# tschnz/Live-Video-Magnification

Hardware: NVIDIA H100
Metric: 1080p frames/sec (Laplace, 6-level) (higher is better)
Workload: dtype f32

## Files before the change

### live-video-magnification_b200/csrc/mc_core.cu

```cuda
#include <algorithm>
#include <cmath>
#include <cstdio>
#include <cstring>
#include <deque>
#include <new>
#include <string>
#include <vector>

#include "../../include/magcore_b200.h"
#include "mc_internal.h"
#include "mc_modes.h"

using namespace mc;

namespace {
thread_local std::string g_create_error;

struct Slot {
    uint8_t *h_in = nullptr, *h_out = nullptr;
    uint8_t *d_in = nullptr, *d_out = nullptr;
    size_t bytes = 0;
    cudaEvent_t ev_in = nullptr, ev_k = nullptr, ev_done = nullptr;
    int produced = 0;
    std::vector<uint8_t> lane_produced;
    uint8_t* user_out = nullptr;
    size_t user_out_step = 0;
    bool direct_out = false;
    int w = 0, h = 0, c = 0;
    bool nv12 = false;
    mc_nv12 user_nv12{};
};
}

struct mc_handle {
    int device = 0;
    int lanes = 1;
    cudaStream_t stream = nullptr, s_in = nullptr, s_out = nullptr;
    DeviceTables tables;
    std::string err;
    uint64_t launches = 0;

    int t_mode = MC_MODE_NONE, t_levels = -1, t_channels = -1, t_w = 0, t_h = 0;
    int t_down = 1, t_roi = 0;
    float t_rx = 0.f, t_ry = 0.f, t_rw = 1.f, t_rh = 1.f;

    bool faithful0 = false, keep_float = false, profile = false, use_tma = true, prefetch_state = true, band_from_state = true, analysis_only = false;
    int ingest_warps = 1;
    int egress_strip = 20;
    int lane_groups = 0;
    Profiler prof;
    int depth = 3;

    MotionMode motion;
    ColorMode color;
    RieszMode riesz;

    float* float_out = nullptr;
    size_t float_out_floats = 0;

    uint8_t *c_raw = nullptr, *c_pre = nullptr, *c_gray = nullptr, *c_out = nullptr;
    size_t c_raw_b = 0, c_pre_b = 0, c_gray_b = 0, c_out_b = 0;
    void* c_tabs = nullptr;
    size_t c_tabs_b = 0;

    uint8_t *k_in = nullptr, *k_out = nullptr;
    size_t k_in_b = 0, k_out_b = 0;

    uint8_t *n_in = nullptr, *n_out = nullptr, *n_flags = nullptr;
    size_t n_in_b = 0, n_out_b = 0, n_flags_b = 0;

    std::vector<Slot> slots;
    std::deque<int> inflight;
    int next_slot = 0;

    std::vector<uint8_t> has_state, hold, ops;
    std::vector<uint8_t> lane_produced;
    uint8_t* d_ops = nullptr;
};

namespace {
thread_local int g_inject_throw = 0;

inline void debug_maybe_throw() {
    if (g_inject_throw > 0 && --g_inject_throw == 0) throw std::bad_alloc();
}

void reset_modes(mc_handle* h);
void tracker_reset(mc_handle* h);

mc_status on_exception(mc_handle* h) noexcept {
    const char* what = "unknown C++ exception";
    std::string buf;
    try { throw; }
    catch (const std::bad_alloc&) { what = "out of host memory (std::bad_alloc)"; }
    catch (const std::exception& e) {
        try { buf = std::string("C++ exception: ") + e.what(); what = buf.c_str(); } catch (...) {}
    }
    catch (...) {}
    try {
        if (h) {
            h->err = what;
// ... 342 lines not shown
    if (h->n_in) cudaFree(h->n_in);
    if (h->n_out) cudaFree(h->n_out);
    if (h->n_flags) cudaFree(h->n_flags);
    if (h->tables.lab_lut) cudaFree(h->tables.lab_lut);
    if (h->tables.inv_gamma) cudaFree(h->tables.inv_gamma);
    if (h->d_ops) cudaFree(h->d_ops);
    if (h->stream) cudaStreamDestroy(h->stream);
    if (h->s_in) cudaStreamDestroy(h->s_in);
    if (h->s_out) cudaStreamDestroy(h->s_out);
    delete h;
} catch (...) {}

void mc_debug_inject_exception(int nth) { g_inject_throw = nth; }

mc_status mc_reset(mc_handle* h) try {
    if (!h) return MC_ERR_INVALID;
    CK(cudaSetDevice(h->device));
    CK(cudaStreamSynchronize(h->stream));
    reset_modes(h);
    tracker_reset(h);
    return MC_OK;
} catch (...) { return on_exception(h); }

mc_status mc_restart_lane(mc_handle* h, int lane) try {
    if (!h) return MC_ERR_INVALID;
    if (lane < 0 || lane >= h->lanes) { h->err = "lane out of range"; return MC_ERR_INVALID; }
    if (h->lanes == 1) return mc_reset(h);
    h->has_state[(size_t)lane] = 0;
    return MC_OK;
} catch (...) { return on_exception(h); }

mc_status mc_hold_lane(mc_handle* h, int lane, int hold) try {
    if (!h) return MC_ERR_INVALID;
    if (lane < 0 || lane >= h->lanes) { h->err = "lane out of range"; return MC_ERR_INVALID; }
    h->hold[(size_t)lane] = hold != 0;
    return MC_OK;
} catch (...) { return on_exception(h); }

mc_status mc_lane_produced(mc_handle* h, uint8_t* produced, int n) try {
    if (!h || !produced) return MC_ERR_INVALID;
    if (n != h->lanes) { h->err = "n must equal the handle's lanes"; return MC_ERR_INVALID; }
    std::memcpy(produced, h->lane_produced.data(), (size_t)n);
    return MC_OK;
} catch (...) { return on_exception(h); }

mc_status mc_set_option(mc_handle* h, const char* key, int value) try {
    if (!h || !key) return MC_ERR_INVALID;
    if (!std::strcmp(key, "faithful_level0")) { h->faithful0 = value != 0; return MC_OK; }
    if (!std::strcmp(key, "keep_float_output")) { h->keep_float = value != 0; return MC_OK; }
    if (!std::strcmp(key, "profile_kernels")) { h->profile = value != 0; return MC_OK; }
    if (!std::strcmp(key, "use_tma")) { h->use_tma = value != 0; return MC_OK; }
    if (!std::strcmp(key, "prefetch_state")) { h->prefetch_state = value != 0; return MC_OK; }
    if (!std::strcmp(key, "lane_groups")) { h->lane_groups = value < 0 ? 0 : value; return MC_OK; }
    if (!std::strcmp(key, "egress_strip")) { h->egress_strip = value == 1 ? 20 : value; return MC_OK; }
    if (!std::strcmp(key, "ingest_warps")) { h->ingest_warps = value; return MC_OK; }
    if (!std::strcmp(key, "band_from_state")) { h->band_from_state = value != 0; return MC_OK; }
    if (!std::strcmp(key, "analysis_only")) { h->analysis_only = value != 0; return MC_OK; }
    if (!std::strcmp(key, "pipeline_depth")) {
        if (value < 1 || value > 16 || !h->inflight.empty()) { h->err = "bad pipeline_depth"; return MC_ERR_INVALID; }
        h->depth = value;
        free_slots(h);
        return MC_OK;
    }
    h->err = std::string("unknown option ") + key;
    return MC_ERR_INVALID;
} catch (...) { return on_exception(h); }

void* mc_stream(mc_handle* h) { return h ? (void*)h->stream : nullptr; }
uint64_t mc_launch_count(mc_handle* h) { return h ? h->launches : 0; }
int mc_pipeline_depth(mc_handle* h) { return h ? h->depth : 0; }

const char* mc_last_error(mc_handle* h) { return h ? h->err.c_str() : g_create_error.c_str(); }

mc_status mc_sync(mc_handle* h) try {
    if (!h) return MC_ERR_INVALID;
    CK(cudaSetDevice(h->device));
    CK(cudaStreamSynchronize(h->stream));
    return MC_OK;
} catch (...) { return on_exception(h); }

mc_status mc_process_device(mc_handle* h, const uint8_t* d_in, int width, int height, int channels, size_t in_step,
                            const mc_params* p, uint8_t* d_out, size_t out_step, int* produced) try {
    if (!h || !produced) return MC_ERR_INVALID;
    CK(cudaSetDevice(h->device));
    return process_device_impl(h, d_in, width, height, channels, in_step, p, d_out, out_step, produced, h->lane_produced.data());
} catch (...) { return on_exception(h); }

mc_status mc_submit(mc_handle* h, const uint8_t* in, int width, int height, int channels, size_t in_step,
                    const mc_params* p, uint8_t* out, size_t out_step) try {
    if (!h || !p) return MC_ERR_INVALID;
    CK(cudaSetDevice(h->device));
    if ((int)h->inflight.size() >= h->depth) { h->err = "pipeline full: call mc_collect first"; return MC_ERR_INVALID; }
    const bool have = in != nullptr && width > 0 && height > 0 && (channels == 1 || channels == 3);
    const size_t row = have ? (size_t)width * channels : 0;
    const size_t bytes = row * (size_t)(have ? height : 0) * h->lanes;
    if (have && in_step < row) { h->err = "step too small"; return MC_ERR_INVALID; }
    mc_status st = ensure_slots(h, std::max<size_t>(bytes, 1));
    if (st != MC_OK) return st;
    const int si = h->next_slot;
    Slot& s = h->slots[(size_t)si];
    s.w = width; s.h = height; s.c = channels; s.produced = 0;
    s.user_out = out; s.user_out_step = out_step; s.direct_out = false; s.nv12 = false;
    if (have && out && out_step < row) { h->err = "out_step too small"; return MC_ERR_INVALID; }
    if (!have) {
        int produced = 0;
        st = process_device_impl(h, nullptr, 0, 0, channels, 0, p, nullptr, 0, &produced, s.lane_produced.data());
        if (st != MC_OK) return st;
// ... 504 lines not shown
```

### live-video-magnification_b200/csrc/mc_laplace.cu

```cuda
#include <cuda.h>

#include "mc_internal.h"
#include "mc_tma.cuh"

namespace mc {

namespace {

__device__ __forceinline__ void prefetch_l1(const void* p) {
#if !defined(MC_CUDA_EMU)
    asm volatile("prefetch.global.L1 [%0];" ::"l"(p));
#else
    (void)p;
#endif
}

constexpr float kInv256 = 1.0f / 256.0f;
constexpr float kInv64 = 1.0f / 64.0f;

__device__ __forceinline__ float down5(float a, float b, float c, float d, float e) {
    return c * 6.0f + (b + d) * 4.0f + a + e;
}

__device__ __forceinline__ float up3(float a, float b, float c) { return __fadd_rn(__fmaf_rn(b, 6.0f, a), c); }
// ... 671 lines not shown
        }
        *reinterpret_cast<float4*>(out + o) = v;
    }
}

constexpr int E2W = 20, E2H = 12;
constexpr int E2P = 20;

struct EgressArgs {
    const uint8_t* in; size_t in_step, in_lane_stride;
    const int16_t* lab; int pitch16; size_t plane16;
    uint8_t* out; size_t out_step, out_lane_stride;
    int w0, h0;
    const float4* gtab; LabInvCoeffs coeffs;
    BandSrc m1; Level l1;
    BandSrc c2; Level l2;
    float chroma;
    float* fout;
    const uint8_t* ops;
    int first_only;
};

__device__ __forceinline__ bool egress_skips(const EgressArgs& a, int lane) {
    const int op = lane_op(a.ops, lane);
    return op == LANE_HOLD || (a.first_only && op == LANE_RUN);
}

template <int C> struct EgressIn;
template <> struct EgressIn<3> { short4 L, A, B; };
template <> struct EgressIn<1> { uint32_t g; };

template <int C>
__device__ __forceinline__ EgressIn<C> egress_load(const EgressArgs& a, int lane, int gy, int gx);
template <>
__device__ __forceinline__ EgressIn<3> egress_load<3>(const EgressArgs& a, int lane, int gy, int gx) {
    const int16_t* lp = a.lab + (size_t)(lane * 3) * a.plane16 + (size_t)gy * a.pitch16 + gx;
    EgressIn<3> r;
    r.L = __ldg(reinterpret_cast<const short4*>(lp));
    r.A = __ldg(reinterpret_cast<const short4*>(lp + a.plane16));
    r.B = __ldg(reinterpret_cast<const short4*>(lp + 2 * a.plane16));
    return r;
}
template <>
__device__ __forceinline__ EgressIn<1> egress_load<1>(const EgressArgs& a, int lane, int gy, int gx) {
    const uint8_t* p = a.in + (size_t)lane * a.in_lane_stride + (size_t)gy * a.in_step + gx;
    EgressIn<1> r;
    r.g = 0;
#pragma unroll
    for (int i = 0; i < 4; ++i)
        if (gx + i < a.w0) r.g |= (uint32_t)__ldg(p + i) << (8 * i);
    return r;
}

template <int C>
__device__ __forceinline__ void egress_convert(const EgressArgs& a, uint8_t* q, float* f, int gx, const EgressIn<C>& in, const float (&up)[C][4]);
template <>
__device__ __forceinline__ void egress_convert<3>(const EgressArgs& a, uint8_t* q, float* f, int gx, const EgressIn<3>& in, const float (&up)[3][4]) {
    uint8_t o8[12];
    float of[12];
    const float chroma64 = a.chroma * kInv64;
    const short vL[4] = {in.L.x, in.L.y, in.L.z, in.L.w}, vA[4] = {in.A.x, in.A.y, in.A.z, in.A.w}, vB[4] = {in.B.x, in.B.y, in.B.z, in.B.w};
#pragma unroll
    for (int i = 0; i < 4; ++i) {
        float L = (float)vL[i] * (100.0f / 16384.0f);
        float A = fmaf((float)vA[i], 1.0f / 64.0f, -128.0f);
        float B = fmaf((float)vB[i], 1.0f / 64.0f, -128.0f);
        if (a.m1.a) {
            L = __fmaf_rn(up[0][i], kInv64, L);
            A = __fadd_rn(A, __fmul_rn(up[1][i], chroma64));
            B = __fadd_rn(B, __fmul_rn(up[2][i], chroma64));
        }
        float ob, og, orr;
        lab_to_bgr_fast(L, A, B, a.coeffs, a.gtab, ob, og, orr);
        of[3 * i] = ob; of[3 * i + 1] = og; of[3 * i + 2] = orr;
        o8[3 * i] = unit01_to_u8(ob); o8[3 * i + 1] = unit01_to_u8(og); o8[3 * i + 2] = unit01_to_u8(orr);
    }
    if (gx + 4 <= a.w0 && ((reinterpret_cast<uintptr_t>(q) & 3) == 0)) {
#pragma unroll
        for (int wd = 0; wd < 3; ++wd)
            reinterpret_cast<uint32_t*>(q)[wd] = (uint32_t)o8[4 * wd] | ((uint32_t)o8[4 * wd + 1] << 8) |
                                                 ((uint32_t)o8[4 * wd + 2] << 16) | ((uint32_t)o8[4 * wd + 3] << 24);
    } else {
#pragma unroll
        for (int i = 0; i < 12; ++i)
            if (gx + i / 3 < a.w0) q[i] = o8[i];
    }
    if (f) {
#pragma unroll
        for (int i = 0; i < 12; ++i)
            if (gx + i / 3 < a.w0) f[i] = of[i];
    }
}
template <>
__device__ __forceinline__ void egress_convert<1>(const EgressArgs& a, uint8_t* q, float* f, int gx, const EgressIn<1>& in, const float (&up)[1][4]) {
    uint8_t o8[4];
    float of[4];
#pragma unroll
    for (int i = 0; i < 4; ++i) {
        float v = u8_to_unit((uint8_t)((in.g >> (8 * i)) & 0xff));
        if (a.m1.a) v = __fmaf_rn(up[0][i], kInv64, v);
        of[i] = v;
        o8[i] = unit_to_u8(v);
    }
    if (gx + 4 <= a.w0 && ((reinterpret_cast<uintptr_t>(q) & 3) == 0)) {
        *reinterpret_cast<uint32_t*>(q) = (uint32_t)o8[0] | ((uint32_t)o8[1] << 8) | ((uint32_t)o8[2] << 16) | ((uint32_t)o8[3] << 24);
    } else {
#pragma unroll
        for (int i = 0; i < 4; ++i)
            if (gx + i < a.w0) q[i] = o8[i];
    }
    if (f) {
#pragma unroll
        for (int i = 0; i < 4; ++i)
            if (gx + i < a.w0) f[i] = of[i];
    }
}

template <int C>
__device__ __forceinline__ void egress_pixels(const EgressArgs& a, int lane, int gy, int gx, const float (&up)[C][4]) {
    const EgressIn<C> in = egress_load<C>(a, lane, gy, gx);
    uint8_t* q = a.out + (size_t)lane * a.out_lane_stride + (size_t)gy * a.out_step + (size_t)gx * C;
    float* f = a.fout ? a.fout + (((size_t)lane * a.h0 + gy) * a.w0 + gx) * C : nullptr;
    egress_convert<C>(a, q, f, gx, in, up);
}

template <int C>
// ... 53 lines not shown
                if (from_state) v[ch] = band_of(v[ch], __ldg(pl[ch] + o1), g1);
            }
            if (has2) {
                const int ky = (y1 >> 1) - by2;
                const bool odd = y1 & 1;
#pragma unroll
                for (int ch = 0; ch < C; ++ch) {
                    const float r0 = sT[ch][ky - 1][j], r1 = sT[ch][ky][j], r2 = sT[ch][ky + 1][j];
                    v[ch] = __fmaf_rn(odd ? up2(r1, r2) : up3(r0, r1, r2), kInv64, v[ch]);
                }
            }
#pragma unroll
            for (int ch = 0; ch < C; ++ch) sD[ch][k][j] = v[ch];
        }
        __syncthreads();
    }
    const int tx = threadIdx.x & 15, ty = threadIdx.x >> 4;
    const int gx = x0 + 4 * tx;
    if (gx >= a.w0) return;
    float up[C][2][4];
    if (a.m1.a) {
#pragma unroll
        for (int ch = 0; ch < C; ++ch) {
            float e[3][4];
#pragma unroll
            for (int q = 0; q < 3; ++q) {
                const float2 p0 = *reinterpret_cast<const float2*>(&sD[ch][ty + q][2 * tx]);
                const float2 p1 = *reinterpret_cast<const float2*>(&sD[ch][ty + q][2 * tx + 2]);
                e[q][0] = up3(p0.x, p0.y, p1.x);
                e[q][1] = up2(p0.y, p1.x);
                e[q][2] = up3(p0.y, p1.x, p1.y);
                e[q][3] = up2(p1.x, p1.y);
            }
#pragma unroll
            for (int i = 0; i < 4; ++i) {
                up[ch][0][i] = up3(e[0][i], e[1][i], e[2][i]);
                up[ch][1][i] = up2(e[1][i], e[2][i]);
            }
        }
    }
#pragma unroll
    for (int ry = 0; ry < 2; ++ry) {
        const int gy = y0 + 2 * ty + ry;
        if (gy >= a.h0) continue;
        float upr[C][4];
#pragma unroll
        for (int ch = 0; ch < C; ++ch)
#pragma unroll
            for (int i = 0; i < 4; ++i) upr[ch][i] = up[ch][ry][i];
        egress_pixels<C>(a, lane, gy, gx, upr);
    }
}

template <int C>
__device__ __forceinline__ EgressIn<C> egress_rows3(const int16_t* const (&p)[C], size_t off);
template <>
__device__ __forceinline__ EgressIn<3> egress_rows3<3>(const int16_t* const (&p)[3], size_t off) {
    EgressIn<3> r;
    r.L = __ldg(reinterpret_cast<const short4*>(p[0] + off));
    r.A = __ldg(reinterpret_cast<const short4*>(p[1] + off));
    r.B = __ldg(reinterpret_cast<const short4*>(p[2] + off));
    return r;
}
template <>
__device__ __forceinline__ EgressIn<1> egress_rows3<1>(const int16_t* const (&)[1], size_t) { return EgressIn<1>{0}; }
template <int C>
__device__ __forceinline__ EgressIn<C> egress_row1(const uint8_t* row, int gx, int w0);
template <>
__device__ __forceinline__ EgressIn<1> egress_row1<1>(const uint8_t* row, int gx, int w0) {
    EgressIn<1> r;
    r.g = 0;
#pragma unroll
    for (int i = 0; i < 4; ++i)
        if (gx >= 0 && gx + i < w0) r.g |= (uint32_t)__ldg(row + gx + i) << (8 * i);
    return r;
}
template <>
__device__ __forceinline__ EgressIn<3> egress_row1<3>(const uint8_t*, int, int) { return EgressIn<3>{}; }

constexpr int EG_ROWS = 64;

template <int C> struct StripM1 { float2 h[C], l[C]; };
template <int C> struct StripH2 { float v[C], vb[C], vr[C], vrb[C]; };

template <int C, int MINB>
__global__ void __launch_bounds__(32, MINB) k_egress_strip(const EgressArgs a) {
    const unsigned full = 0xffffffffu;
    const int lane_id = threadIdx.x;
    const int lane = blockIdx.z;
    const int gx = blockIdx.x * DS_COLS - 4 + lane_id * 4;
    const int f0 = blockIdx.y * EG_ROWS;
    if (f0 >= a.h0 || egress_skips(a, lane)) return;
    const int f_end = min(f0 + EG_ROWS, a.h0);
    const bool px_owner = lane_id >= 1 && lane_id <= 30 && gx < a.w0;
    if (!a.m1.a) {
        float zero[C][4];
#pragma unroll
        for (int ch = 0; ch < C; ++ch)
#pragma unroll
            for (int i = 0; i < 4; ++i) zero[ch][i] = 0.0f;
        if (px_owner)
            for (int gy = f0; gy < f_end; ++gy) egress_pixels<C>(a, lane, gy, gx, zero);
        return;
    }
    const int w1 = a.l1.w, h1 = a.l1.h, w2 = a.l2.w, h2 = a.l2.h;
    const int x1a = gx >> 1, x2 = gx >> 2;
    const bool has2 = a.c2.a != nullptr, from_state = a.m1.b != nullptr, st2 = a.c2.b != nullptr;
    const float g1 = a.m1.gain, g2 = a.c2.gain;
    const int x1l = x1a < 0 ? 0 : (x1a >= w1 ? ((w1 - 1) & ~1) : x1a);
    const int x2l = x2 < 0 ? 0 : (x2 >= w2 ? w2 - 1 : x2);
    const int x2r = x2l + 1 >= w2 ? w2 - 1 : x2l + 1;
    const int gxl = px_owner ? gx : 0;
    size_t base1[C], base2[C];
#pragma unroll
    for (int ch = 0; ch < C; ++ch) {
        base1[ch] = (size_t)(lane * C + ch) * a.l1.plane + x1l;
        base2[ch] = (size_t)(lane * C + ch) * a.l2.plane;
    }

    auto row1 = [&](int y1) { return (size_t)(y1 < h1 ? y1 : h1 - 1) * a.l1.pitch; };
    auto ld_m1 = [&](int y1) {
        StripM1<C> m;
        const size_t ro = row1(y1);
#pragma unroll
        for (int ch = 0; ch < C; ++ch) {
            m.h[ch] = __ldg(reinterpret_cast<const float2*>(a.m1.a + base1[ch] + ro));
            m.l[ch] = from_state ? __ldg(reinterpret_cast<const float2*>(a.m1.b + base1[ch] + ro)) : make_float2(0.f, 0.f);
        }
        return m;
    };
    auto pf_m1 = [&](int y1) {
        const size_t ro = row1(y1);
#pragma unroll
        for (int ch = 0; ch < C; ++ch) {
            prefetch_l1(a.m1.a + base1[ch] + ro);
            if (from_state) prefetch_l1(a.m1.b + base1[ch] + ro);
        }
    };
    auto ld_h2 = [&](int y2) {
        StripH2<C> r;
        const size_t ro = (size_t)upsrc(y2, h2) * a.l2.pitch;
#pragma unroll
        for (int ch = 0; ch < C; ++ch) {
            r.v[ch] = r.vb[ch] = r.vr[ch] = r.vrb[ch] = 0.f;
            if (has2) {
                r.v[ch] = __ldg(a.c2.a + base2[ch] + ro + x2l);
                if (st2) r.vb[ch] = __ldg(a.c2.b + base2[ch] + ro + x2l);
                if (lane_id == 31) {
                    r.vr[ch] = __ldg(a.c2.a + base2[ch] + ro + x2r);
                    if (st2) r.vrb[ch] = __ldg(a.c2.b + base2[ch] + ro + x2r);
                }
            }
        }
        return r;
    };
    auto pf_h2 = [&](int y2) {
        const size_t ro = (size_t)upsrc(y2, h2) * a.l2.pitch;
        if (has2) {
#pragma unroll
            for (int ch = 0; ch < C; ++ch) {
                prefetch_l1(a.c2.a + base2[ch] + ro + x2l);
                if (st2) prefetch_l1(a.c2.b + base2[ch] + ro + x2l);
            }
        }
    };
    auto pf_in = [&](int gy) {
        if (C == 3) {
            const int16_t* lp = a.lab + (size_t)(lane * 3) * a.plane16 + (size_t)gy * a.pitch16 + gxl;
            prefetch_l1(lp); prefetch_l1(lp + a.plane16); prefetch_l1(lp + 2 * a.plane16);
        } else {
            prefetch_l1(a.in + (size_t)lane * a.in_lane_stride + (size_t)gy * a.in_step + gxl);
        }
    };
    __shared__ float2 sH[3][C][32];
    __shared__ float4 sE[3][C][32];
    auto slot = [](int r) { return (r + 3) % 3; };
    auto expand_h2 = [&](const StripH2<C>& in, int i) {
        const int sl = slot(i);
#pragma unroll
        for (int ch = 0; ch < C; ++ch) {
            const float v = st2 ? band_of(in.v[ch], in.vb[ch], g2) : in.v[ch];
            float l = __shfl_up_sync(full, v, 1), r = __shfl_down_sync(full, v, 1);
            if (lane_id == 31) r = st2 ? band_of(in.vr[ch], in.vrb[ch], g2) : in.vr[ch];
            if (x2 == 0) l = r;
            if (x2 + 1 >= w2) r = v;
            sH[sl][ch][lane_id] = make_float2(up3(l, v, r), up2(v, r));
        }
    };
    auto cur1_row = [&](const StripM1<C>& m, int y1, float (&E)[C][4]) {
        const bool odd = y1 & 1;
        const int i = y1 >> 1;
        const int sp = slot(odd ? i : i - 1), sq = slot(odd ? i + 1 : i), sr = slot(i + 1);
#pragma unroll
        for (int ch = 0; ch < C; ++ch) {
            float ca = m.h[ch].x, cb = m.h[ch].y;
            if (from_state) {
                ca = band_of(ca, m.l[ch].x, g1);
                cb = band_of(cb, m.l[ch].y, g1);
            }
            if (has2) {
                const float2 p = sH[sp][ch][lane_id], q = sH[sq][ch][lane_id], r = sH[sr][ch][lane_id];
                ca = __fmaf_rn(odd ? up2(p.x, q.x) : up3(p.x, q.x, r.x), kInv64, ca);
                cb = __fmaf_rn(odd ? up2(p.y, q.y) : up3(p.y, q.y, r.y), kInv64, cb);
            }
            if (x1a + 1 >= w1) cb = ca;
            float left = __shfl_up_sync(full, cb, 1), right = __shfl_down_sync(full, ca, 1);
            if (x1a == 0) left = cb;
            if (x1a + 2 >= w1) right = cb;
            E[ch][0] = up3(left, ca, cb);
            E[ch][1] = up2(ca, cb);
            E[ch][2] = up3(ca, cb, right);
            E[ch][3] = up2(cb, right);
        }
    };
    auto put_E = [&](int j, const float (&E)[C][4]) {
        const int sl = slot(j);
#pragma unroll
        for (int ch = 0; ch < C; ++ch) sE[sl][ch][lane_id] = make_float4(E[ch][0], E[ch][1], E[ch][2], E[ch][3]);
    };

    const int j0 = f0 >> 1;
    {
        const int ic = j0 >> 1;
        const StripH2<C> ra = ld_h2(ic - 1), rb = ld_h2(ic), rc = ld_h2(ic + 1);
        const StripM1<C> mp = ld_m1(j0 > 0 ? j0 - 1 : 1), m0 = ld_m1(j0);
        pf_m1(j0 + 1);
        pf_in(2 * j0);
        pf_in(min(2 * j0 + 1, a.h0 - 1));
        expand_h2(ra, ic - 1);
        expand_h2(rb, ic);
        expand_h2(rc, ic + 1);
        float E[C][4];
        if (j0 > 0) { cur1_row(mp, j0 - 1, E); put_E(j0 - 1, E); }
        cur1_row(m0, j0, E);
        put_E(j0, E);
    }
    const int j_end = (f_end + 1) >> 1;
    const size_t st1 = (size_t)a.l1.pitch, st16 = (size_t)a.pitch16;
    const float* ph[C];
    const float* pl[C];
    const int16_t* pin[C];
#pragma unroll
    for (int ch = 0; ch < C; ++ch) {
        const size_t ro = row1(j0 + 1);
        ph[ch] = a.m1.a + base1[ch] + ro;
        pl[ch] = from_state ? a.m1.b + base1[ch] + ro : ph[ch];
        pin[ch] = C == 3 ? a.lab + (size_t)(lane * 3 + ch) * a.plane16 + (size_t)(2 * j0) * st16 + gxl : nullptr;
    }
    const uint8_t* pg = C == 1 ? a.in + (size_t)lane * a.in_lane_stride + (size_t)(2 * j0) * a.in_step : nullptr;
    uint8_t* pq = a.out + (size_t)lane * a.out_lane_stride + (size_t)(2 * j0) * a.out_step + (size_t)gx * C;
    int sm = slot(j0 - 1), s0 = slot(j0), sp = slot(j0 + 1);
    for (int j = j0; j < j_end; ++j) {
        const int jn = j + 1;
        const bool two = 2 * j + 1 < f_end;
        StripM1<C> cm;
#pragma unroll
        for (int ch = 0; ch < C; ++ch) {
            cm.h[ch] = __ldg(reinterpret_cast<const float2*>(ph[ch]));
            cm.l[ch] = from_state ? __ldg(reinterpret_cast<const float2*>(pl[ch])) : make_float2(0.f, 0.f);
        }
        StripH2<C> chh;
        if (!(jn & 1) && jn < h1) chh = ld_h2((jn >> 1) + 1);
        EgressIn<C> in0, in1;
        if (C == 3) {
            in0 = egress_rows3<C>(pin, 0);
            in1 = egress_rows3<C>(pin, two ? st16 : 0);
        } else {
            in0 = egress_row1<C>(pg, gx, a.w0);
            in1 = egress_row1<C>(two ? pg + a.in_step : pg, gx, a.w0);
        }
        if (jn < j_end) {
            const bool adv1 = jn + 1 < h1;
            if (jn & 1) pf_h2(((jn + 1) >> 1) + 1);
#pragma unroll
            for (int ch = 0; ch < C; ++ch) {
                if (adv1) { ph[ch] += st1; pl[ch] += st1; }
                prefetch_l1(ph[ch]);
                if (from_state) prefetch_l1(pl[ch]);
                if (C == 3) {
                    pin[ch] += 2 * st16;
                    prefetch_l1(pin[ch]);
                    if (2 * jn + 1 < a.h0) prefetch_l1(pin[ch] + st16);
                }
            }
            if (C == 1) { pg += 2 * a.in_step; prefetch_l1(pg + gxl); }
        }
        float Ep[C][4];
        if (jn >= h1) {
#pragma unroll
            for (int ch = 0; ch < C; ++ch) {
                const float4 e = sE[s0][ch][lane_id];
                Ep[ch][0] = e.x; Ep[ch][1] = e.y; Ep[ch][2] = e.z; Ep[ch][3] = e.w;
            }
        } else {
            if (!(jn & 1)) expand_h2(chh, (jn >> 1) + 1);
            cur1_row(cm, jn, Ep);
        }
#pragma unroll
        for (int ch = 0; ch < C; ++ch) sE[sp][ch][lane_id] = make_float4(Ep[ch][0], Ep[ch][1], Ep[ch][2], Ep[ch][3]);
        if (j == 0) {
#pragma unroll
            for (int ch = 0; ch < C; ++ch) sE[sm][ch][lane_id] = make_float4(Ep[ch][0], Ep[ch][1], Ep[ch][2], Ep[ch][3]);
        }
        if (px_owner) {
            float up[C][4], t0[C][4];
#pragma unroll
            for (int ch = 0; ch < C; ++ch) {
                const float4 em = sE[sm][ch][lane_id], e0 = sE[s0][ch][lane_id];
                t0[ch][0] = e0.x; t0[ch][1] = e0.y; t0[ch][2] = e0.z; t0[ch][3] = e0.w;
                up[ch][0] = up3(em.x, e0.x, Ep[ch][0]);
                up[ch][1] = up3(em.y, e0.y, Ep[ch][1]);
                up[ch][2] = up3(em.z, e0.z, Ep[ch][2]);
                up[ch][3] = up3(em.w, e0.w, Ep[ch][3]);
            }
            float* f = a.fout ? a.fout + (((size_t)lane * a.h0 + 2 * j) * a.w0 + gx) * C : nullptr;
            egress_convert<C>(a, pq, f, gx, in0, up);
            if (two) {
#pragma unroll
                for (int ch = 0; ch < C; ++ch)
#pragma unroll
                    for (int i = 0; i < 4; ++i) up[ch][i] = up2(t0[ch][i], Ep[ch][i]);
                egress_convert<C>(a, pq + a.out_step, f ? f + (size_t)a.w0 * C : nullptr, gx, in1, up);
            }
        }
        pq += 2 * a.out_step;
        const int t = sm; sm = s0; s0 = sp; sp = t;
    }
}

__global__ void k_copy(float* __restrict__ dst, const float* __restrict__ src, size_t n) {
    for (size_t i = (size_t)blockIdx.x * blockDim.x + threadIdx.x; i < n; i += (size_t)gridDim.x * blockDim.x)
        dst[i] = src[i];
}

inline unsigned cdiv(int a, int b) { return (unsigned)((a + b - 1) / b); }

}

typedef CUresult (*TensorMapEncodeFn)(CUtensorMap*, CUtensorMapDataType, cuuint32_t, void*, const cuuint64_t*, const cuuint64_t*,
                                      const cuuint32_t*, const cuuint32_t*, CUtensorMapInterleave, CUtensorMapSwizzle,
                                      CUtensorMapL2promotion, CUtensorMapFloatOOBfill);
static TensorMapEncodeFn tensor_map_encoder() {
    static const TensorMapEncodeFn fn = [] {
        void* p = nullptr;
        cudaDriverEntryPointQueryResult qres;
        if (cudaGetDriverEntryPoint("cuTensorMapEncodeTiled", &p, cudaEnableDefault, &qres) != cudaSuccess || !p) {
            cudaGetLastError();
            p = nullptr;
        }
        return reinterpret_cast<TensorMapEncodeFn>(p);
    }();
    return fn;
}

bool make_tensor_map_box(void* out_map, const float* base, const Level& l, int planes, int box_w, int box_h) {
    const TensorMapEncodeFn encode = tensor_map_encoder();
    if (!encode) return false;
    const cuuint64_t dims[3] = {(cuuint64_t)l.w, (cuuint64_t)l.h, (cuuint64_t)planes};
    const cuuint64_t strides[2] = {(cuuint64_t)l.pitch * sizeof(float), (cuuint64_t)l.plane * sizeof(float)};
    const cuuint32_t box[3] = {(cuuint32_t)box_w, (cuuint32_t)box_h, 1u};
    const cuuint32_t estr[3] = {1u, 1u, 1u};
    const CUresult r = encode(reinterpret_cast<CUtensorMap*>(out_map), CU_TENSOR_MAP_DATA_TYPE_FLOAT32, 3, const_cast<float*>(base),
                              dims, strides, box, estr, CU_TENSOR_MAP_INTERLEAVE_NONE, CU_TENSOR_MAP_SWIZZLE_NONE,
                              CU_TENSOR_MAP_L2_PROMOTION_L2_128B, CU_TENSOR_MAP_FLOAT_OOB_FILL_NONE);
    return r == CUDA_SUCCESS;
}

bool make_level_tensor_map(void* out_map, const float* base, const Level& l, int planes, bool state_tile) {
    return make_tensor_map_box(out_map, base, l, planes, state_tile ? TW : GW, state_tile ? TH : GH);
}

cudaError_t launch_lab16(const FrameIO& io, const DeviceTables& tb, int16_t* lab, int pitch16, size_t plane16,
                         cudaStream_t s, float* l_f32, int l_pitch, size_t l_plane) {
    const int aligned = (reinterpret_cast<uintptr_t>(io.in) % 4 == 0) && (io.in_step % 4 == 0) && (io.in_lane_stride % 4 == 0);
    dim3 grid(cdiv(cdiv(io.w, 4), 256), io.h, io.lanes);
    k_lab16<<<grid, 256, 0, s>>>(io.in, io.in_step, io.in_lane_stride, io.w, io.h, tb.lab_lut, lab, pitch16, plane16, aligned, l_f32, l_pitch, l_plane, io.ops);
    return cudaGetLastError();
}
// ... 25 lines not shown
    k.ops = a.ops;
    k.in_vec_ok = a.in_kind == IN_U8 ? ((reinterpret_cast<uintptr_t>(a.g) % 4 == 0) && (a.in_row % 4 == 0) && (a.in_plane % 4 == 0)) : 1;
    return k;
}

cudaError_t launch_level_clip(const LevelArgs& a, int frames, cudaStream_t s) {
    const LevelKArgs k = level_kargs(a);
    dim3 grid(cdiv(a.lf.w, TW), cdiv(a.lf.h, TH), a.planes);
    static const CUtensorMap dummy{};
    const CUtensorMap* tg = reinterpret_cast<const CUtensorMap*>(a.tmap);
    if (a.in_kind == IN_F32 && tg) k_level_clip<IN_F32, true><<<grid, 256, 0, s>>>(k, frames, a.planes, *tg);
    else if (a.in_kind == IN_F32) k_level_clip<IN_F32, false><<<grid, 256, 0, s>>>(k, frames, a.planes, dummy);
    else if (a.in_kind == IN_LAB16) k_level_clip<IN_LAB16, false><<<grid, 256, 0, s>>>(k, frames, a.planes, dummy);
    else k_level_clip<IN_U8, false><<<grid, 256, 0, s>>>(k, frames, a.planes, dummy);
    return cudaGetLastError();
}

cudaError_t launch_level(const LevelArgs& a, cudaStream_t s) {
    const LevelKArgs k = level_kargs(a);
    dim3 grid(cdiv(a.lf.w, TW), cdiv(a.lf.h, TH), a.planes);
    static const CUtensorMap dummy{};
    const CUtensorMap* tg = reinterpret_cast<const CUtensorMap*>(a.tmap);
    if (a.in_kind == IN_F32 && tg && a.tmap_hi && a.tmap_lo)
        k_level<IN_F32, true, true><<<grid, 256, 0, s>>>(k, *tg, *reinterpret_cast<const CUtensorMap*>(a.tmap_hi),
                                                          *reinterpret_cast<const CUtensorMap*>(a.tmap_lo));
    else if (a.in_kind == IN_F32 && tg) k_level<IN_F32, true, false><<<grid, 256, 0, s>>>(k, *tg, dummy, dummy);
    else if (a.in_kind == IN_F32) k_level<IN_F32, false, false><<<grid, 256, 0, s>>>(k, dummy, dummy, dummy);
    else if (a.in_kind == IN_LAB16) k_level<IN_LAB16, false, false><<<grid, 256, 0, s>>>(k, dummy, dummy, dummy);
    else k_level<IN_U8, false, false><<<grid, 256, 0, s>>>(k, dummy, dummy, dummy);
    return cudaGetLastError();
}

cudaError_t launch_down(const LevelArgs& a, cudaStream_t s) {
    DownArgs k;
    k.g = a.g; k.in_plane = a.in_plane; k.in_row = a.in_row; k.channels = a.channels;
    for (int i = 0; i < 3; ++i) { k.sc[i] = a.sc[i]; k.of[i] = a.of[i]; }
    k.lf = a.lf; k.lc = a.lc; k.g_next = a.g_next;
    k.ops = a.ops;
    k.in_vec_ok = a.in_kind == IN_U8 ? ((reinterpret_cast<uintptr_t>(a.g) % 4 == 0) && (a.in_row % 4 == 0) && (a.in_plane % 4 == 0)) : 1;
    dim3 grid(cdiv(a.lf.w, DS_COLS), cdiv(a.lc.h, DS_ROWS * DS_WARPS), a.planes);
    if (a.in_kind == IN_F32) k_down_strip<IN_F32><<<grid, 32 * DS_WARPS, 0, s>>>(k);
    else if (a.in_kind == IN_LAB16) k_down_strip<IN_LAB16><<<grid, 32 * DS_WARPS, 0, s>>>(k);
    else k_down_strip<IN_U8><<<grid, 32 * DS_WARPS, 0, s>>>(k);
    return cudaGetLastError();
}

cudaError_t launch_collapse(const Level& lf, const Level& lc, const BandSrc& fine, const BandSrc& coarse, float* out, int planes,
                            cudaStream_t s, const uint8_t* ops, int channels) {
    dim3 grid(cdiv(lf.w, TW), cdiv(lf.h, TH), planes);
    k_collapse<<<grid, 256, 0, s>>>(lf, lc, fine, coarse, out, ops, channels);
    return cudaGetLastError();
}

cudaError_t launch_egress(const FrameIO& io, const DeviceTables& tb, const int16_t* lab, int pitch16, size_t plane16,
                          const BandSrc& m1, const Level& l1, const BandSrc& c2, const Level& l2, float chroma,
                          float* fout, cudaStream_t s, int strip, bool first_only) {
    EgressArgs a;
    a.in = io.in; a.in_step = io.in_step; a.in_lane_stride = io.in_lane_stride;
    a.lab = lab; a.pitch16 = pitch16; a.plane16 = plane16;
    a.out = io.out; a.out_step = io.out_step; a.out_lane_stride = io.out_lane_stride;
    a.w0 = io.w; a.h0 = io.h;
    a.gtab = tb.inv_gamma; a.coeffs = tb.inv_coeffs;
    a.m1 = m1; a.l1 = l1; a.c2 = c2; a.l2 = l2; a.chroma = chroma; a.fout = fout;
    a.ops = io.ops; a.first_only = first_only ? 1 : 0;
    if (strip) {
        dim3 grid(cdiv(io.w, DS_COLS), cdiv(io.h, EG_ROWS), io.lanes);
        if (io.channels != 3) k_egress_strip<1, 24><<<grid, 32, 0, s>>>(a);
        else if (strip == 16) k_egress_strip<3, 16><<<grid, 32, 0, s>>>(a);
        else if (strip == 24) k_egress_strip<3, 24><<<grid, 32, 0, s>>>(a);
        else k_egress_strip<3, 20><<<grid, 32, 0, s>>>(a);
    } else {
        dim3 grid(cdiv(io.w, TW), cdiv(io.h, TH), io.lanes);
        if (io.channels == 3) k_egress<3><<<grid, 256, 0, s>>>(a);
        else k_egress<1><<<grid, 256, 0, s>>>(a);
    }
    return cudaGetLastError();
}

cudaError_t launch_copy_planes(float* dst, const float* src, size_t n, cudaStream_t s) {
    unsigned blocks = (unsigned)((n + 255) / 256);
    if (blocks > 132 * 8) blocks = 132 * 8;
    if (blocks == 0) blocks = 1;
    k_copy<<<blocks, 256, 0, s>>>(dst, src, n);
    return cudaGetLastError();
}

}
```

Measured before the change: 17040.

## Restructure egress strip kernel with warp-uniform dark-gamma fallback and int offsets

Reworks the strip egress kernel. Gamma is now computed with a fast exp2/log2 path, and the spline table lookup runs only when some lane in the warp has a dark value, checked with a warp vote. Pointer arithmetic moves to 32-bit offsets, the float output path becomes a compile-time template flag, and all lanes compute the upsampled values uniformly to avoid divergence. The default strip launch bound also changes from 20 to 16; the risk is extra register pressure and a possible change in numeric behaviour near the dark threshold.

```diff
diff --git a/live-video-magnification_b200/csrc/mc_core.cu b/live-video-magnification_b200/csrc/mc_core.cu
--- a/live-video-magnification_b200/csrc/mc_core.cu
+++ b/live-video-magnification_b200/csrc/mc_core.cu
@@ -46,7 +46,7 @@
 
     bool faithful0 = false, keep_float = false, profile = false, use_tma = true, prefetch_state = true, band_from_state = true, analysis_only = false;
     int ingest_warps = 1;
-    int egress_strip = 20;
+    int egress_strip = 16;
     int lane_groups = 0;
     Profiler prof;
     int depth = 3;
@@ -495,7 +495,7 @@
     if (!std::strcmp(key, "use_tma")) { h->use_tma = value != 0; return MC_OK; }
     if (!std::strcmp(key, "prefetch_state")) { h->prefetch_state = value != 0; return MC_OK; }
     if (!std::strcmp(key, "lane_groups")) { h->lane_groups = value < 0 ? 0 : value; return MC_OK; }
-    if (!std::strcmp(key, "egress_strip")) { h->egress_strip = value == 1 ? 20 : value; return MC_OK; }
+    if (!std::strcmp(key, "egress_strip")) { h->egress_strip = value == 1 ? 16 : value; return MC_OK; }
     if (!std::strcmp(key, "ingest_warps")) { h->ingest_warps = value; return MC_OK; }
     if (!std::strcmp(key, "band_from_state")) { h->band_from_state = value != 0; return MC_OK; }
     if (!std::strcmp(key, "analysis_only")) { h->analysis_only = value != 0; return MC_OK; }
diff --git a/live-video-magnification_b200/csrc/mc_laplace.cu b/live-video-magnification_b200/csrc/mc_laplace.cu
--- a/live-video-magnification_b200/csrc/mc_laplace.cu
+++ b/live-video-magnification_b200/csrc/mc_laplace.cu
@@ -747,6 +747,53 @@
     return r;
 }
 
+__device__ __forceinline__ void egress_lab_in(short l, short av, short bv, bool motion, float u0, float u1, float u2,
+                                              float chroma64, float& L, float& A, float& B) {
+    L = (float)l * (100.0f / 16384.0f);
+    A = fmaf((float)av, 1.0f / 64.0f, -128.0f);
+    B = fmaf((float)bv, 1.0f / 64.0f, -128.0f);
+    if (motion) {
+        L = __fmaf_rn(u0, kInv64, L);
+        A = __fadd_rn(A, __fmul_rn(u1, chroma64));
+        B = __fadd_rn(B, __fmul_rn(u2, chroma64));
+    }
+}
+
+constexpr float kGammaDark = 8.0f / 1024.0f;
+
+__device__ __forceinline__ void lab_lin(float L, float a, float b, const LabInvCoeffs& k, float& vb, float& vg, float& vr) {
+    const float y_lin = L * (1.0f / 903.3f);
+    const float fy_lin = 7.787f * y_lin + 16.0f / 116.0f;
+    const float fy_cub = (L + 16.0f) * (1.0f / 116.0f);
+    const bool lo = L <= 8.0f;
+    const float fy = lo ? fy_lin : fy_cub;
+    const float Y = lo ? y_lin : fy_cub * fy_cub * fy_cub;
+    const float fx = a * (1.0f / 500.0f) + fy;
+    const float fz = fy - b * (1.0f / 200.0f);
+    const float fth = 6.0f / 29.0f;
+    const float X = fx <= fth ? (fx - 16.0f / 116.0f) * (1.0f / 7.787f) : fx * fx * fx;
+    const float Z = fz <= fth ? (fz - 16.0f / 116.0f) * (1.0f / 7.787f) : fz * fz * fz;
+    vb = __saturatef(__fmaf_rn(k.c[2], Z, __fmaf_rn(k.c[1], Y, __fmul_rn(k.c[0], X))));
+    vg = __saturatef(__fmaf_rn(k.c[5], Z, __fmaf_rn(k.c[3], X, __fmul_rn(k.c[4], Y))));
+    vr = __saturatef(__fmaf_rn(k.c[8], Z, __fmaf_rn(k.c[6], X, __fmul_rn(k.c[7], Y))));
+}
+
+__device__ __forceinline__ float gamma_fast(float v) { return fmaf(1.055f, mc_ex2(mc_lg2(v) * (1.0f / 2.4f)), -0.055f); }
+
+__device__ __forceinline__ void lab_to_bgr_egress(float L, float a, float b, const LabInvCoeffs& k, const float4* __restrict__ gtab,
+                                                  float& ob, float& og, float& orr) {
+    float vb, vg, vr;
+    lab_lin(L, a, b, k, vb, vg, vr);
+    ob = gamma_fast(vb);
+    og = gamma_fast(vg);
+    orr = gamma_fast(vr);
+    if (fminf(vb, fminf(vg, vr)) < kGammaDark) {
+        if (vb < kGammaDark) ob = spline_gamma(vb, gtab);
+        if (vg < kGammaDark) og = spline_gamma(vg, gtab);
+        if (vr < kGammaDark) orr = spline_gamma(vr, gtab);
+    }
+}
+
 template <int C>
 __device__ __forceinline__ void egress_convert(const EgressArgs& a, uint8_t* q, float* f, int gx, const EgressIn<C>& in, const float (&up)[C][4]);
 template <>
@@ -757,16 +804,10 @@
     const short vL[4] = {in.L.x, in.L.y, in.L.z, in.L.w}, vA[4] = {in.A.x, in.A.y, in.A.z, in.A.w}, vB[4] = {in.B.x, in.B.y, in.B.z, in.B.w};
 #pragma unroll
     for (int i = 0; i < 4; ++i) {
-        float L = (float)vL[i] * (100.0f / 16384.0f);
-        float A = fmaf((float)vA[i], 1.0f / 64.0f, -128.0f);
-        float B = fmaf((float)vB[i], 1.0f / 64.0f, -128.0f);
-        if (a.m1.a) {
-            L = __fmaf_rn(up[0][i], kInv64, L);
-            A = __fadd_rn(A, __fmul_rn(up[1][i], chroma64));
-            B = __fadd_rn(B, __fmul_rn(up[2][i], chroma64));
-        }
+        float L, A, B;
+        egress_lab_in(vL[i], vA[i], vB[i], a.m1.a != nullptr, up[0][i], up[1][i], up[2][i], chroma64, L, A, B);
         float ob, og, orr;
-        lab_to_bgr_fast(L, A, B, a.coeffs, a.gtab, ob, og, orr);
+        lab_to_bgr_egress(L, A, B, a.coeffs, a.gtab, ob, og, orr);
         of[3 * i] = ob; of[3 * i + 1] = og; of[3 * i + 2] = orr;
         o8[3 * i] = unit01_to_u8(ob); o8[3 * i + 1] = unit01_to_u8(og); o8[3 * i + 2] = unit01_to_u8(orr);
     }
@@ -926,22 +967,7 @@
     }
 }
 
-template <int C>
-__device__ __forceinline__ EgressIn<C> egress_rows3(const int16_t* const (&p)[C], size_t off);
-template <>
-__device__ __forceinline__ EgressIn<3> egress_rows3<3>(const int16_t* const (&p)[3], size_t off) {
-    EgressIn<3> r;
-    r.L = __ldg(reinterpret_cast<const short4*>(p[0] + off));
-    r.A = __ldg(reinterpret_cast<const short4*>(p[1] + off));
-    r.B = __ldg(reinterpret_cast<const short4*>(p[2] + off));
-    return r;
-}
-template <>
-__device__ __forceinline__ EgressIn<1> egress_rows3<1>(const int16_t* const (&)[1], size_t) { return EgressIn<1>{0}; }
-template <int C>
-__device__ __forceinline__ EgressIn<C> egress_row1(const uint8_t* row, int gx, int w0);
-template <>
-__device__ __forceinline__ EgressIn<1> egress_row1<1>(const uint8_t* row, int gx, int w0) {
+__device__ __forceinline__ EgressIn<1> egress_row1(const uint8_t* row, int gx, int w0) {
     EgressIn<1> r;
     r.g = 0;
 #pragma unroll
@@ -949,15 +975,86 @@
         if (gx >= 0 && gx + i < w0) r.g |= (uint32_t)__ldg(row + gx + i) << (8 * i);
     return r;
 }
-template <>
-__device__ __forceinline__ EgressIn<3> egress_row1<3>(const uint8_t*, int, int) { return EgressIn<3>{}; }
 
 constexpr int EG_ROWS = 64;
 
 template <int C> struct StripM1 { float2 h[C], l[C]; };
 template <int C> struct StripH2 { float v[C], vb[C], vr[C], vrb[C]; };
 
-template <int C, int MINB>
+__device__ __forceinline__ bool warp_any(bool p) {
+#if defined(MC_CUDA_EMU)
+    int v = p ? 1 : 0;
+    for (int m = 16; m; m >>= 1) v |= __shfl_xor_sync(0xffffffffu, v, m);
+    return v != 0;
+#else
+    return __any_sync(0xffffffffu, p);
+#endif
+}
+
+template <int C> struct StripPx { uint32_t w[C]; float v[4 * C], f[4 * C]; bool dark; };
+
+template <int C>
+__device__ __forceinline__ StripPx<C> strip_px(const EgressArgs& a, float chroma64, const EgressIn<C>& in, const float (&up)[C][4]) {
+    StripPx<C> o;
+    uint32_t b[4 * C];
+    if constexpr (C == 3) {
+        const short vL[4] = {in.L.x, in.L.y, in.L.z, in.L.w}, vA[4] = {in.A.x, in.A.y, in.A.z, in.A.w}, vB[4] = {in.B.x, in.B.y, in.B.z, in.B.w};
+        float lo = 1.0f;
+#pragma unroll
+        for (int i = 0; i < 4; ++i) {
+            float L, A, B;
+            egress_lab_in(vL[i], vA[i], vB[i], true, up[0][i], up[1][i], up[2][i], chroma64, L, A, B);
+            lab_lin(L, A, B, a.coeffs, o.v[3 * i], o.v[3 * i + 1], o.v[3 * i + 2]);
+            lo = fminf(lo, fminf(o.v[3 * i], fminf(o.v[3 * i + 1], o.v[3 * i + 2])));
+        }
+#pragma unroll
+        for (int k = 0; k < 12; ++k) {
+            o.f[k] = gamma_fast(o.v[k]);
+            b[k] = unit01_to_u8(o.f[k]);
+        }
+        o.dark = lo < kGammaDark;
+    } else {
+#pragma unroll
+        for (int i = 0; i < 4; ++i) {
+            o.f[i] = __fmaf_rn(up[0][i], kInv64, u8_to_unit((uint8_t)((in.g >> (8 * i)) & 0xff)));
+            b[i] = unit_to_u8(o.f[i]);
+        }
+        o.dark = false;
+    }
+#pragma unroll
+    for (int wd = 0; wd < C; ++wd) o.w[wd] = b[4 * wd] | (b[4 * wd + 1] << 8) | (b[4 * wd + 2] << 16) | (b[4 * wd + 3] << 24);
+    return o;
+}
+
+template <int C>
+__device__ __forceinline__ void strip_dark(const float4* __restrict__ gtab, StripPx<C>& o) {
+#pragma unroll
+    for (int k = 0; k < 4 * C; ++k)
+        if (o.v[k] < kGammaDark) {
+            o.f[k] = spline_gamma(o.v[k], gtab);
+            const int sh = 8 * (k & 3);
+            o.w[k >> 2] = (o.w[k >> 2] & ~(0xffu << sh)) | ((uint32_t)unit01_to_u8(o.f[k]) << sh);
+        }
+}
+
+template <int C, bool FOUT>
+__device__ __forceinline__ void strip_store(const StripPx<C>& o, uint8_t* q, float* f, int gx, int w0, bool words, bool bytes) {
+    if (words) {
+#pragma unroll
+        for (int wd = 0; wd < C; ++wd) reinterpret_cast<uint32_t*>(q)[wd] = o.w[wd];
+    } else if (bytes) {
+#pragma unroll
+        for (int i = 0; i < 4 * C; ++i)
+            if (gx + i / C < w0) q[i] = (uint8_t)(o.w[i >> 2] >> (8 * (i & 3)));
+    }
+    if (FOUT && (words || bytes)) {
+#pragma unroll
+        for (int i = 0; i < 4 * C; ++i)
+            if (gx + i / C < w0) f[i] = o.f[i];
+    }
+}
+
+template <int C, int MINB, bool FOUT>
 __global__ void __launch_bounds__(32, MINB) k_egress_strip(const EgressArgs a) {
     const unsigned full = 0xffffffffu;
     const int lane_id = threadIdx.x;
@@ -985,63 +1082,61 @@
     const int x2l = x2 < 0 ? 0 : (x2 >= w2 ? w2 - 1 : x2);
     const int x2r = x2l + 1 >= w2 ? w2 - 1 : x2l + 1;
     const int gxl = px_owner ? gx : 0;
-    size_t base1[C], base2[C];
-#pragma unroll
-    for (int ch = 0; ch < C; ++ch) {
-        base1[ch] = (size_t)(lane * C + ch) * a.l1.plane + x1l;
-        base2[ch] = (size_t)(lane * C + ch) * a.l2.plane;
-    }
-
-    auto row1 = [&](int y1) { return (size_t)(y1 < h1 ? y1 : h1 - 1) * a.l1.pitch; };
-    auto ld_m1 = [&](int y1) {
+    const size_t pl1 = a.l1.plane, pl2 = a.l2.plane, pl16 = a.plane16;
+    const float* const m1a = a.m1.a + (size_t)(lane * C) * pl1;
+    const float* const m1b = from_state ? a.m1.b + (size_t)(lane * C) * pl1 : m1a;
+    const float* const c2a = has2 ? a.c2.a + (size_t)(lane * C) * pl2 : a.m1.a;
+    const float* const c2b = st2 ? a.c2.b + (size_t)(lane * C) * pl2 : c2a;
+    const int16_t* const lab = C == 3 ? a.lab + (size_t)(lane * 3) * pl16 : nullptr;
+
+    auto row1 = [&](int y1) { return (y1 < h1 ? y1 : h1 - 1) * a.l1.pitch; };
+    auto ld_m1 = [&](int o) {
         StripM1<C> m;
-        const size_t ro = row1(y1);
 #pragma unroll
         for (int ch = 0; ch < C; ++ch) {
-            m.h[ch] = __ldg(reinterpret_cast<const float2*>(a.m1.a + base1[ch] + ro));
-            m.l[ch] = from_state ? __ldg(reinterpret_cast<const float2*>(a.m1.b + base1[ch] + ro)) : make_float2(0.f, 0.f);
+            m.h[ch] = __ldg(reinterpret_cast<const float2*>(m1a + ch * pl1 + o));
+            m.l[ch] = from_state ? __ldg(reinterpret_cast<const float2*>(m1b + ch * pl1 + o)) : make_float2(0.f, 0.f);
         }
         return m;
     };
-    auto pf_m1 = [&](int y1) {
-        const size_t ro = row1(y1);
+    auto pf_m1 = [&](int o) {
 #pragma unroll
         for (int ch = 0; ch < C; ++ch) {
-            prefetch_l1(a.m1.a + base1[ch] + ro);
-            if (from_state) prefetch_l1(a.m1.b + base1[ch] + ro);
+            prefetch_l1(m1a + ch * pl1 + o);
+            if (from_state) prefetch_l1(m1b + ch * pl1 + o);
         }
     };
     auto ld_h2 = [&](int y2) {
         StripH2<C> r;
-        const size_t ro = (size_t)upsrc(y2, h2) * a.l2.pitch;
+        const int ro = upsrc(y2, h2) * a.l2.pitch;
 #pragma unroll
         for (int ch = 0; ch < C; ++ch) {
             r.v[ch] = r.vb[ch] = r.vr[ch] = r.vrb[ch] = 0.f;
             if (has2) {
-                r.v[ch] = __ldg(a.c2.a + base2[ch] + ro + x2l);
-                if (st2) r.vb[ch] = __ldg(a.c2.b + base2[ch] + ro + x2l);
+                r.v[ch] = __ldg(c2a + ch * pl2 + ro + x2l);
+                if (st2) r.vb[ch] = __ldg(c2b + ch * pl2 + ro + x2l);
                 if (lane_id == 31) {
-                    r.vr[ch] = __ldg(a.c2.a + base2[ch] + ro + x2r);
-                    if (st2) r.vrb[ch] = __ldg(a.c2.b + base2[ch] + ro + x2r);
+                    r.vr[ch] = __ldg(c2a + ch * pl2 + ro + x2r);
+                    if (st2) r.vrb[ch] = __ldg(c2b + ch * pl2 + ro + x2r);
                 }
             }
         }
         return r;
     };
     auto pf_h2 = [&](int y2) {
-        const size_t ro = (size_t)upsrc(y2, h2) * a.l2.pitch;
+        const int ro = upsrc(y2, h2) * a.l2.pitch + x2l;
         if (has2) {
 #pragma unroll
             for (int ch = 0; ch < C; ++ch) {
-                prefetch_l1(a.c2.a + base2[ch] + ro + x2l);
-                if (st2) prefetch_l1(a.c2.b + base2[ch] + ro + x2l);
+                prefetch_l1(c2a + ch * pl2 + ro);
+                if (st2) prefetch_l1(c2b + ch * pl2 + ro);
             }
         }
     };
     auto pf_in = [&](int gy) {
         if (C == 3) {
-            const int16_t* lp = a.lab + (size_t)(lane * 3) * a.plane16 + (size_t)gy * a.pitch16 + gxl;
-            prefetch_l1(lp); prefetch_l1(lp + a.plane16); prefetch_l1(lp + 2 * a.plane16);
+            const int16_t* lp = lab + gy * a.pitch16 + gxl;
+            prefetch_l1(lp); prefetch_l1(lp + pl16); prefetch_l1(lp + 2 * pl16);
         } else {
             prefetch_l1(a.in + (size_t)lane * a.in_lane_stride + (size_t)gy * a.in_step + gxl);
         }
@@ -1097,8 +1192,8 @@
     {
         const int ic = j0 >> 1;
         const StripH2<C> ra = ld_h2(ic - 1), rb = ld_h2(ic), rc = ld_h2(ic + 1);
-        const StripM1<C> mp = ld_m1(j0 > 0 ? j0 - 1 : 1), m0 = ld_m1(j0);
-        pf_m1(j0 + 1);
+        const StripM1<C> mp = ld_m1(row1(j0 > 0 ? j0 - 1 : 1) + x1l), m0 = ld_m1(row1(j0) + x1l);
+        pf_m1(row1(j0 + 1) + x1l);
         pf_in(2 * j0);
         pf_in(min(2 * j0 + 1, a.h0 - 1));
         expand_h2(ra, ic - 1);
@@ -1110,54 +1205,53 @@
         put_E(j0, E);
     }
     const int j_end = (f_end + 1) >> 1;
-    const size_t st1 = (size_t)a.l1.pitch, st16 = (size_t)a.pitch16;
-    const float* ph[C];
-    const float* pl[C];
-    const int16_t* pin[C];
-#pragma unroll
-    for (int ch = 0; ch < C; ++ch) {
-        const size_t ro = row1(j0 + 1);
-        ph[ch] = a.m1.a + base1[ch] + ro;
-        pl[ch] = from_state ? a.m1.b + base1[ch] + ro : ph[ch];
-        pin[ch] = C == 3 ? a.lab + (size_t)(lane * 3 + ch) * a.plane16 + (size_t)(2 * j0) * st16 + gxl : nullptr;
-    }
+    const int st1 = a.l1.pitch, st16 = a.pitch16;
+    int o1 = row1(j0 + 1) + x1l;
+    int o16 = 2 * j0 * st16 + gxl;
     const uint8_t* pg = C == 1 ? a.in + (size_t)lane * a.in_lane_stride + (size_t)(2 * j0) * a.in_step : nullptr;
     uint8_t* pq = a.out + (size_t)lane * a.out_lane_stride + (size_t)(2 * j0) * a.out_step + (size_t)gx * C;
+    float* pf = FOUT ? a.fout + (((size_t)lane * a.h0 + 2 * j0) * a.w0 + gx) * C : nullptr;
+    const bool words = px_owner && gx + 4 <= a.w0 &&
+                       ((reinterpret_cast<uintptr_t>(a.out + (size_t)lane * a.out_lane_stride) | a.out_step) & 3) == 0;
+    const bool bytes = px_owner && !words;
+    const float chroma64 = a.chroma * kInv64;
     int sm = slot(j0 - 1), s0 = slot(j0), sp = slot(j0 + 1);
     for (int j = j0; j < j_end; ++j) {
         const int jn = j + 1;
         const bool two = 2 * j + 1 < f_end;
-        StripM1<C> cm;
-#pragma unroll
-        for (int ch = 0; ch < C; ++ch) {
-            cm.h[ch] = __ldg(reinterpret_cast<const float2*>(ph[ch]));
-            cm.l[ch] = from_state ? __ldg(reinterpret_cast<const float2*>(pl[ch])) : make_float2(0.f, 0.f);
-        }
+        const StripM1<C> cm = ld_m1(o1);
         StripH2<C> chh;
         if (!(jn & 1) && jn < h1) chh = ld_h2((jn >> 1) + 1);
         EgressIn<C> in0, in1;
-        if (C == 3) {
-            in0 = egress_rows3<C>(pin, 0);
-            in1 = egress_rows3<C>(pin, two ? st16 : 0);
+        if constexpr (C == 3) {
+            const int16_t* p = lab + o16;
+            in0.L = __ldg(reinterpret_cast<const short4*>(p));
+            in0.A = __ldg(reinterpret_cast<const short4*>(p + pl16));
+            in0.B = __ldg(reinterpret_cast<const short4*>(p + 2 * pl16));
+            if (two) p += st16;
+            in1.L = __ldg(reinterpret_cast<const short4*>(p));
+            in1.A = __ldg(reinterpret_cast<const short4*>(p + pl16));
+            in1.B = __ldg(reinterpret_cast<const short4*>(p + 2 * pl16));
         } else {
-            in0 = egress_row1<C>(pg, gx, a.w0);
-            in1 = egress_row1<C>(two ? pg + a.in_step : pg, gx, a.w0);
+            in0 = egress_row1(pg, gx, a.w0);
+            in1 = egress_row1(two ? pg + a.in_step : pg, gx, a.w0);
         }
         if (jn < j_end) {
-            const bool adv1 = jn + 1 < h1;
             if (jn & 1) pf_h2(((jn + 1) >> 1) + 1);
-#pragma unroll
-            for (int ch = 0; ch < C; ++ch) {
-                if (adv1) { ph[ch] += st1; pl[ch] += st1; }
-                prefetch_l1(ph[ch]);
-                if (from_state) prefetch_l1(pl[ch]);
-                if (C == 3) {
-                    pin[ch] += 2 * st16;
-                    prefetch_l1(pin[ch]);
-                    if (2 * jn + 1 < a.h0) prefetch_l1(pin[ch] + st16);
+            if (jn + 1 < h1) o1 += st1;
+            pf_m1(o1);
+            if constexpr (C == 3) {
+                o16 += 2 * st16;
+                const bool nxt = 2 * jn + 1 < a.h0;
+#pragma unroll
+                for (int ch = 0; ch < C; ++ch) {
+                    prefetch_l1(lab + ch * pl16 + o16);
+                    if (nxt) prefetch_l1(lab + ch * pl16 + o16 + st16);
                 }
-            }
-            if (C == 1) { pg += 2 * a.in_step; prefetch_l1(pg + gxl); }
+            } else {
+                pg += 2 * a.in_step;
+                prefetch_l1(pg + gxl);
+            }
         }
         float Ep[C][4];
         if (jn >= h1) {
@@ -1176,28 +1270,31 @@
 #pragma unroll
             for (int ch = 0; ch < C; ++ch) sE[sm][ch][lane_id] = make_float4(Ep[ch][0], Ep[ch][1], Ep[ch][2], Ep[ch][3]);
         }
-        if (px_owner) {
-            float up[C][4], t0[C][4];
-#pragma unroll
-            for (int ch = 0; ch < C; ++ch) {
-                const float4 em = sE[sm][ch][lane_id], e0 = sE[s0][ch][lane_id];
-                t0[ch][0] = e0.x; t0[ch][1] = e0.y; t0[ch][2] = e0.z; t0[ch][3] = e0.w;
-                up[ch][0] = up3(em.x, e0.x, Ep[ch][0]);
-                up[ch][1] = up3(em.y, e0.y, Ep[ch][1]);
-                up[ch][2] = up3(em.z, e0.z, Ep[ch][2]);
-                up[ch][3] = up3(em.w, e0.w, Ep[ch][3]);
-            }
-            float* f = a.fout ? a.fout + (((size_t)lane * a.h0 + 2 * j) * a.w0 + gx) * C : nullptr;
-            egress_convert<C>(a, pq, f, gx, in0, up);
-            if (two) {
-#pragma unroll
-                for (int ch = 0; ch < C; ++ch)
-#pragma unroll
-                    for (int i = 0; i < 4; ++i) up[ch][i] = up2(t0[ch][i], Ep[ch][i]);
-                egress_convert<C>(a, pq + a.out_step, f ? f + (size_t)a.w0 * C : nullptr, gx, in1, up);
-            }
+        float up0[C][4], up1[C][4];
+#pragma unroll
+        for (int ch = 0; ch < C; ++ch) {
+            const float4 em = sE[sm][ch][lane_id], e0 = sE[s0][ch][lane_id];
+            up0[ch][0] = up3(em.x, e0.x, Ep[ch][0]);
+            up0[ch][1] = up3(em.y, e0.y, Ep[ch][1]);
+            up0[ch][2] = up3(em.z, e0.z, Ep[ch][2]);
+            up0[ch][3] = up3(em.w, e0.w, Ep[ch][3]);
+            up1[ch][0] = up2(e0.x, Ep[ch][0]);
+            up1[ch][1] = up2(e0.y, Ep[ch][1]);
+            up1[ch][2] = up2(e0.z, Ep[ch][2]);
+            up1[ch][3] = up2(e0.w, Ep[ch][3]);
+        }
+        {
+            StripPx<C> o = strip_px<C>(a, chroma64, in0, up0);
+            if (C == 3 && warp_any(px_owner && o.dark)) strip_dark<C>(a.gtab, o);
+            strip_store<C, FOUT>(o, pq, pf, gx, a.w0, words, bytes);
+        }
+        {
+            StripPx<C> o = strip_px<C>(a, chroma64, in1, up1);
+            if (C == 3 && warp_any(px_owner && o.dark)) strip_dark<C>(a.gtab, o);
+            strip_store<C, FOUT>(o, pq + a.out_step, FOUT ? pf + (size_t)a.w0 * C : nullptr, gx, a.w0, two && words, two && bytes);
         }
         pq += 2 * a.out_step;
+        if (FOUT) pf += (size_t)(2 * a.w0) * C;
         const int t = sm; sm = s0; s0 = sp; sp = t;
     }
 }
@@ -1329,6 +1426,12 @@
     return cudaGetLastError();
 }
 
+template <int C, int MINB>
+static void launch_egress_strip(const EgressArgs& a, dim3 grid, cudaStream_t s) {
+    if (a.fout) k_egress_strip<C, C == 3 ? 16 : MINB, true><<<grid, 32, 0, s>>>(a);
+    else k_egress_strip<C, MINB, false><<<grid, 32, 0, s>>>(a);
+}
+
 cudaError_t launch_egress(const FrameIO& io, const DeviceTables& tb, const int16_t* lab, int pitch16, size_t plane16,
                           const BandSrc& m1, const Level& l1, const BandSrc& c2, const Level& l2, float chroma,
                           float* fout, cudaStream_t s, int strip, bool first_only) {
@@ -1342,10 +1445,10 @@
     a.ops = io.ops; a.first_only = first_only ? 1 : 0;
     if (strip) {
         dim3 grid(cdiv(io.w, DS_COLS), cdiv(io.h, EG_ROWS), io.lanes);
-        if (io.channels != 3) k_egress_strip<1, 24><<<grid, 32, 0, s>>>(a);
-        else if (strip == 16) k_egress_strip<3, 16><<<grid, 32, 0, s>>>(a);
-        else if (strip == 24) k_egress_strip<3, 24><<<grid, 32, 0, s>>>(a);
-        else k_egress_strip<3, 20><<<grid, 32, 0, s>>>(a);
+        if (io.channels != 3) launch_egress_strip<1, 24>(a, grid, s);
+        else if (strip == 16) launch_egress_strip<3, 16>(a, grid, s);
+        else if (strip == 24) launch_egress_strip<3, 24>(a, grid, s);
+        else launch_egress_strip<3, 20>(a, grid, s);
     } else {
         dim3 grid(cdiv(io.w, TW), cdiv(io.h, TH), io.lanes);
         if (io.channels == 3) k_egress<3><<<grid, 256, 0, s>>>(a);
```

After: 17900, median of 6. 1.05x the previous value.
